# mark1222/arena

Hardware: AMD Instinct MI355X
Metric: mnist_mlp_train_throughput (higher is better)
Workload: dtype fp32; 1 GPU; model=mnist_mlp_784-500-10 (relu, dropout 0.9, adam 1e-3), global_batch=100, parallelism=dp1, impl=fused, exec=hipgraph[full,1 steps/graph]; timed: 2479/2479 graph-replayed, 0 eager, launch=single

## Files before the change

csrc/ops/mlp_kernels.hip:

```cpp
#include "common.h"
#include "adam.h"

#include <algorithm>
#include <cmath>

using namespace arena;

#ifndef ARENA_EXP
#define ARENA_EXP 0
#endif
#ifdef ARENA_TIMELINE
__device__ long long arena::arena_tl_buf[4 * ARENA_TL_BLOCKS * ARENA_TL_SLOTS];
extern "C" hipError_t arena_timeline_read(long long* host, int clear) {
  const size_t bytes = sizeof(long long) * 4 * ARENA_TL_BLOCKS * ARENA_TL_SLOTS;
  hipError_t e = hipDeviceSynchronize();
  if (e == hipSuccess) e = hipMemcpyFromSymbol(host, HIP_SYMBOL(arena::arena_tl_buf), bytes);
  if (e == hipSuccess && clear) {
    void* p = nullptr;
    e = hipGetSymbolAddress(&p, HIP_SYMBOL(arena::arena_tl_buf));
    if (e == hipSuccess) e = hipMemset(p, 0, bytes);
  }
  return e;
}
#endif
// ... 100 lines not shown
#pragma unroll
  for (int r = 0; r < 4; ++r) red[w][4 * g + r][c] = acc[r];
  __syncthreads();
  for (int t = threadIdx.x; t < 256; t += WAVES * 64) {
    const int rr = t >> 4, cc = t & 15;
    const int gm = m0 + rr, gn = n0 + cc;
    if (gm < M && gn < N) {
      float v = 0.f;
#pragma unroll
      for (int ww = 0; ww < WAVES; ++ww) v += red[ww][rr][cc];
      v += bv;
      if (act == 1) v = fmaxf(v, 0.f);
      if (keep_thr != 0xFFFFFFFFu) {
        const uint32_t h = hash4(seed, step, (uint32_t)gm, (uint32_t)gn);
        v = (h < keep_thr) ? v * inv_keep : 0.f;
      }
      Y[(long long)gm * N + gn] = v;
    }
  }
}

constexpr int kHeadMaxT = 16;
constexpr int kHeadMaxC = 16;
constexpr int kHeadStage = 16;

template <int LT, int STAGE, int CB, int TB>
__global__ __launch_bounds__(256) __attribute__((amdgpu_waves_per_eu(1, 4))) void xent_head_kernel(
    const float* __restrict__ H, int M, int D, const float* __restrict__ W2,
    const float* __restrict__ b2, int C, ArenaRowSource lab, float* __restrict__ dlogits,
    float* __restrict__ dZ, float inv_keep, int relu_mask, float loss_scale,
    float* __restrict__ loss_acc, int* __restrict__ correct_acc, int hist_len,
    const long long* hist_step, ArenaCounterOp ctr) {
  extern __shared__ __attribute__((aligned(16))) float ws[];
  const int lane = lane_id();
  const int r = blockIdx.x * 4 + wave_id();
  const int rc = min(r, M - 1);
  const long long pr = gather_row(make_gather(lab), rc);
  int y;
  if constexpr (LT == 1) y = (int)static_cast<const uint8_t*>(lab.ptr)[pr];
  else if constexpr (LT == 2) y = static_cast<const int*>(lab.ptr)[pr];
  else y = (int)static_cast<const long long*>(lab.ptr)[pr];
  float h[TB];
#pragma unroll
  for (int t = 0; t < TB; ++t) h[t] = H[(long long)rc * D + min(lane + 64 * t, D - 1)];
  const int n4 = (D * C) >> 2;
  float4 st[STAGE];
#pragma unroll
  for (int i = 0; i < STAGE; ++i)
    st[i] = reinterpret_cast<const float4*>(W2)[min((int)threadIdx.x + 256 * i, n4 - 1)];
  const float bl = b2 ? b2[min(lane, C - 1)] : 0.f;
  const long long hs = hist_step ? *hist_step : 0;
#pragma unroll
  for (int i = 0; i < STAGE; ++i) {
    const int q = threadIdx.x + 256 * i;
    reinterpret_cast<float4*>(ws)[q < n4 ? q : n4] = st[i];
  }
  counter_op(ctr);
  const int hmask = hist_len - 1;
  const int slot = (int)hs & hmask;
  if (hist_len > 1 && blockIdx.x == 0 && threadIdx.x == 0) {
    const int nxt = (int)(hs + 1) & hmask;
    loss_acc[nxt] = 0.f;
    correct_acc[nxt] = 0;
  }
  __syncthreads();
  if (r >= M) return;
  int jo[TB];
#pragma unroll
  for (int t = 0; t < TB; ++t) {
    const int j = lane + 64 * t;
    jo[t] = min(j, D - 1);
    h[t] = (j < D) ? h[t] : 0.f;
  }

  float lg[CB];
#pragma unroll
  for (int cc = 0; cc < CB; ++cc) {
    const float* wr = ws + min(cc, C - 1) * D;
    float s = 0.f;
#pragma unroll
    for (int t = 0; t < TB; ++t) s += h[t] * wr[jo[t]];
    lg[cc] = s;
  }
#pragma unroll
  for (int cc = 0; cc < CB; ++cc) {
    const float tot = wave_sum_fast(lg[cc]) +
                      __int_as_float(__builtin_amdgcn_readlane(__float_as_int(bl), cc));
    lg[cc] = (cc < C) ? tot : -INFINITY;
  }
  float mx = lg[0];
  int arg = 0;
#pragma unroll
  for (int cc = 1; cc < CB; ++cc) {
    const bool gt = lg[cc] > mx;
    mx = gt ? lg[cc] : mx;
    arg = gt ? cc : arg;
  }
  float se = 0.f;
#pragma unroll
  for (int cc = 0; cc < CB; ++cc) se += (cc < C) ? hw_exp2((lg[cc] - mx) * kLog2e) : 0.f;
  const float lse = mx + hw_log2(se) * kLn2;
  float ly = 0.f;
#pragma unroll
  for (int cc = 0; cc < CB; ++cc) ly = (cc == y) ? lg[cc] : ly;
  if (lane == 0) {
    atomicAdd(&loss_acc[slot], (lse - ly) * loss_scale);
    atomicAdd(&correct_acc[slot], arg == y ? 1 : 0);
  }
  if (dlogits == nullptr) return;

  float gcl[CB];
#pragma unroll
  for (int cc = 0; cc < CB; ++cc)
    gcl[cc] = (cc < C) ? (hw_exp2((lg[cc] - lse) * kLog2e) - (cc == y ? 1.f : 0.f)) * loss_scale
                       : 0.f;
  if (lane < C) {
    float v = 0.f;
#pragma unroll
    for (int cc = 0; cc < CB; ++cc) v = (cc == lane) ? gcl[cc] : v;
    dlogits[(long long)r * C + lane] = v;
  }
  if (dZ == nullptr) return;
  float o[TB];
#pragma unroll
  for (int t = 0; t < TB; ++t) {
    float s = 0.f;
#pragma unroll
    for (int cc = 0; cc < CB; ++cc) s += gcl[cc] * ws[min(cc, C - 1) * D + jo[t]];
    o[t] = relu_mask ? ((h[t] > 0.f) ? s * inv_keep : 0.f) : s;
  }
#pragma unroll
  for (int t = 0; t < TB; ++t) {
    const int j = lane + 64 * t;
    if (j < D) dZ[(long long)r * D + j] = o[t];
  }
}

constexpr int kMaxProblems = 2;
struct WGradArgs {
  ArenaWGradProblem p[kMaxProblems];
  int nprob;
  ArenaAdam adam;
  float grad_scale;
  ArenaCounterOp ctr;
  ArenaHead head;
  int head_block;
};

constexpr int kMC = 128;
constexpr int kXsStride = 80;
constexpr int kXItems = (kMC * 16) / 256;
constexpr int kZItems = (kMC * 4) / 256;
constexpr int kDItems = (kMC * 16) / 256;

__device__ __forceinline__ void lds_barrier() {
  asm volatile("s_waitcnt lgkmcnt(0)" ::: "memory");
  __builtin_amdgcn_s_barrier();
  asm volatile("" ::: "memory");
}

template <int XT>
__device__ __forceinline__ void load_x_items(const ArenaWGradProblem& P, const Gather& gt, int mc0,
                                             int mcn, int k0, float4 (&v)[kXItems]) {
  int prow[kXItems];
#pragma unroll
  for (int i = 0; i < kXItems; ++i) {
    const int t = threadIdx.x + 256 * i;
    prow[i] = gather_row(gt, mc0 + min(t >> 4, mcn - 1));
  }
#pragma unroll
  for (int i = 0; i < kXItems; ++i) {
    const int q = (threadIdx.x + 256 * i) & 15;
    float f[4];
    load4<XT>(P.x, prow[i], min(k0 + 4 * q, P.K - 4), f);
    v[i] = make_float4(f[0], f[1], f[2], f[3]);
  }
}

__device__ __forceinline__ int load_label(const ArenaRowSource& lab, long long pr) {
  if (lab.dtype == 1) return (int)static_cast<const uint8_t*>(lab.ptr)[pr];
  if (lab.dtype == 2) return static_cast<const int*>(lab.ptr)[pr];
  return (int)static_cast<const long long*>(lab.ptr)[pr];
}

template <int SPEC>
struct WSpec {
  static constexpr bool known = SPEC != 0;
  static constexpr int s = SPEC - 1;
  static constexpr int xt = s & 1, hm = (s >> 1) & 3, gather = (s >> 3) & 1, mode = (s >> 4) & 1;
  static constexpr bool sp = known && ((s >> 5) & 1);
};


constexpr int wgrad_spec(int xt, int hm, int gather, int mode, int sp = 0) {
  return 1 + xt + 2 * hm + 8 * gather + 16 * mode + 32 * sp;
}

template <int CB, int SPEC, int LG, int LDT>
__device__ __forceinline__ void wgrad_body(const WGradArgs& args, int pi, float* Xs, float* Zs,
                                           float* Ds, float* W2s, int* Ys, float* B2s) {
  using WS = WSpec<SPEC>;
  const ArenaWGradProblem& P = args.p[pi];
  const ArenaHead& HD = args.head;
  const int local = blockIdx.x - P.block_begin;
  int tn, tk;
  if ((P.tiles_n & 7) == 0 && (P.block_begin & 7) == 0) {
    const int xcd = local & 7, slot = local >> 3;
    tn = xcd + 8 * (slot / P.tiles_k);
    tk = slot % P.tiles_k;
  } else {
    tn = local / P.tiles_k;
    tk = local % P.tiles_k;
  }
  const int n0 = tn * 16, k0 = tk * 64;
  const int lane = lane_id(), w = wave_id();
  const int g = lane >> 4, c = lane & 15;
  const int kk = k0 + 16 * w + c;
  const int kkc = min(kk, P.K - 1);
  const bool bias_wave = (tk == 0) && (w == 0);
  const int mode = WS::known ? WS::mode : P.mode;
  const int xt = WS::known ? WS::xt : P.xt;
  const int hmode = WS::known ? WS::hm : P.hd_mode;
  const bool has_bias = mode == 1 ? P.pB != nullptr : P.gB != nullptr;
  const Gather gt = (WS::known && !WS::gather) ? Gather{nullptr, 0, P.M} : make_gather(P.x);
  const bool zvec = (P.N & 3) == 0;
  ARENA_TL(1, 0);
  int lz;
  asm volatile("v_mov_b32 %0, 0" : "=v"(lz));
  long long hstep_raw = 0, adam_t = 1;
  float adam_lr = args.adam.lr;
  if constexpr (WS::known) {
    if (WS::hm) hstep_raw = *reinterpret_cast<const int*>(HD.step) + lz;
    if (WS::mode == 1) {
      adam_t = *reinterpret_cast<const int*>(args.adam.t_ptr) + lz;
      adam_lr = *args.adam.lr_ptr + __int_as_float(lz);
    }
  } else {
    if (hmode) hstep_raw = *HD.step;
    if (mode == 1) {
      adam_t = args.adam.t_ptr ? *args.adam.t_ptr : 1;
      adam_lr = args.adam.lr_ptr ? *args.adam.lr_ptr : args.adam.lr;
    }
  }
  const float* logits = nullptr;
  long long hstep = 0;

  f32x4 acc = {0.f, 0.f, 0.f, 0.f};
  f32x4 accb = {0.f, 0.f, 0.f, 0.f};
  float pw[4], mw[4], vw[4], pb[4], mb[4], vb[4];
  const int nchunks = WS::known ? 1 : (P.M + kMC - 1) / kMC;
  for (int ci = 0; ci < nchunks; ++ci) {
    const int mc0 = ci * kMC;
    const int mcn = min(kMC, P.M - mc0);
    float4 xv[kXItems];
    if (ARENA_EXP & 2) {
#pragma unroll
      for (int i = 0; i < kXItems; ++i) xv[i] = make_float4(0.5f, 0.25f, 0.f, 1.f);
    } else if (xt == 1) {
      load_x_items<1>(P, gt, mc0, mcn, k0, xv);
    } else {
      load_x_items<0>(P, gt, mc0, mcn, k0, xv);
    }
    ARENA_TL(1, 8);
    float4 zv[kZItems];
    float dv[kDItems];
    float wv = 0.f, bv = 0.f;
    int yv = 0;
    if (hmode == 0) {
#pragma unroll
      for (int i = 0; i < kZItems; ++i) {
        const int t = threadIdx.x + 256 * i;
        const int rr = min(t >> 2, mcn - 1), q = t & 3;
        const int n = n0 + 4 * q;
        const float* srcp = P.dz + (long long)(mc0 + rr) * P.N;
        if (zvec) {
          zv[i] = *reinterpret_cast<const float4*>(srcp + min(n, P.N - 4));
        } else {
          zv[i] = make_float4(srcp[min(n, P.N - 1)], srcp[min(n + 1, P.N - 1)],
                              srcp[min(n + 2, P.N - 1)], srcp[min(n + 3, P.N - 1)]);
        }
      }
    } else {
      const int C = HD.C;
      if ((int)threadIdx.x < kMC) {
        const Gather lg = (LG == 0) ? Gather{nullptr, 0, P.M} : make_gather(HD.lab);
        const long long pr = gather_row(lg, mc0 + min((int)threadIdx.x, mcn - 1));
        if constexpr (LDT == 1) yv = static_cast<const uint8_t*>(HD.lab.ptr)[pr];
        else if constexpr (LDT == 2) yv = static_cast<const int*>(HD.lab.ptr)[pr];
        else yv = load_label(HD.lab, pr);
      }
      {
        const float* b2p = HD.b2 ? HD.b2 : P.hd_w2 ? P.hd_w2 : HD.logits2;
        const float b2v = b2p[min((int)threadIdx.x & 15, C - 1)];
        bv = HD.b2 ? b2v : 0.f;
      }
      if (hmode == 2) {
#pragma unroll
        for (int i = 0; i < kZItems; ++i) {
          const int t = threadIdx.x + 256 * i;
          const int rr = min(t >> 2, mcn - 1), q = t & 3;
          if (ARENA_EXP & 4) zv[i] = make_float4(1.f, 0.f, 1.f, 1.f);
          else zv[i] = *reinterpret_cast<const float4*>(P.hd_h + (long long)(mc0 + rr) * P.N +
                                                        min(n0 + 4 * q, P.N - 4));
        }
        wv = P.hd_w2[(long long)min((int)threadIdx.x >> 4, C - 1) * P.N +
                     min(n0 + ((int)threadIdx.x & 15), P.N - 1)];
      }
      ARENA_TL(1, 9);
      if (mc0 == 0) {
        if constexpr (WS::sp) {
          logits = HD.logits2 + (long long)HD.parity * P.M * HD.C;
          ARENA_TL(1, 1);
        } else {
          if (ARENA_EXP & 16) hstep_raw = 7;
          hstep = hstep_raw + HD.step_off;
          logits = HD.logits2 + (long long)(hstep & 1) * P.M * HD.C;
          ARENA_TL_DEP((int)hstep);
          ARENA_TL(1, 1);
        }
      }
#pragma unroll
      for (int i = 0; i < kDItems; ++i) {
        const int t = threadIdx.x + 256 * i;
        if (ARENA_EXP & 1) dv[i] = 0.01f * (float)(t & 15);
        else dv[i] = logits[(long long)(mc0 + min(t >> 4, mcn - 1)) * C + min(t & 15, C - 1)];
      }
      ARENA_TL(1, 10);
      if (mc0 == 0 && (int)blockIdx.x == args.head_block) {
        if constexpr (WS::sp) hstep = hstep_raw + HD.step_off;
        float* nxt = HD.logits2 + (long long)((hstep + 1) & 1) * P.M * HD.C;
        for (int i = threadIdx.x; i < P.M * HD.C; i += 256) nxt[i] = 0.f;
        if (HD.nr_out != nullptr && (int)threadIdx.x < HD.nr_batch) {
          long long q = mod_fp64((double)(hstep + 1) * (double)HD.nr_batch, HD.nr_len) +
                        (long long)threadIdx.x;
          q = (q >= HD.nr_len) ? q - HD.nr_len : q;
          HD.nr_out[threadIdx.x] = HD.nr_perm[q];
        }
        if (threadIdx.x == 0 && HD.hist_len > 1) {
          const int ns = (int)(hstep + 1) & (HD.hist_len - 1);
          HD.loss_acc[ns] = 0.f;
          HD.correct_acc[ns] = 0;
        }
      }
    }
    if (mc0 == 0 && mode == 1 && (ARENA_EXP & 32)) {
#pragma unroll
      for (int r = 0; r < 4; ++r) { pw[r] = 0.1f; mw[r] = 0.01f; vw[r] = 0.001f; }
#pragma unroll
      for (int r = 0; r < 4; ++r) { pb[r] = 0.1f; mb[r] = 0.01f; vb[r] = 0.001f; }
    } else if (mc0 == 0 && mode == 1) {
#pragma unroll
      for (int r = 0; r < 4; ++r) {
        const long long off = (long long)min(n0 + 4 * g + r, P.N - 1) * P.K + kkc;
        pw[r] = P.pW[off]; mw[r] = P.mW[off]; vw[r] = P.vW[off];
      }
      {
        const float* pbp = has_bias ? P.pB : P.pW;
        const float* mbp = has_bias ? P.mB : P.mW;
        const float* vbp = has_bias ? P.vB : P.vW;
#pragma unroll
        for (int r = 0; r < 4; ++r) {
          const int n = min(n0 + 4 * g + r, P.N - 1);
          pb[r] = pbp[n]; mb[r] = mbp[n]; vb[r] = vbp[n];
        }
      }
    }
#pragma unroll
    for (int i = 0; i < kXItems; ++i) {
      const int t = threadIdx.x + 256 * i;
      const int rr = t >> 4, q = t & 15;
      const float4 o = (k0 + 4 * q < P.K) ? xv[i] : make_float4(0.f, 0.f, 0.f, 0.f);
      *reinterpret_cast<float4*>(&Xs[rr * kXsStride + 4 * q]) = o;
    }
    if (hmode == 0) {
#pragma unroll
      for (int i = 0; i < kZItems; ++i) {
        const int t = threadIdx.x + 256 * i;
        const int rr = t >> 2, q = t & 3;
        const int n = n0 + 4 * q;
        float4 o = zv[i];
        o.x = (n + 0 < P.N) ? o.x : 0.f;
        o.y = (n + 1 < P.N) ? o.y : 0.f;
        o.z = (n + 2 < P.N) ? o.z : 0.f;
        o.w = (n + 3 < P.N) ? o.w : 0.f;
        if (rr >= mcn) o = make_float4(0.f, 0.f, 0.f, 0.f);
        *reinterpret_cast<float4*>(&Zs[rr * 16 + 4 * q]) = o;
      }
    } else {
      const int C = HD.C;
#pragma unroll
      for (int i = 0; i < kDItems; ++i) Ds[threadIdx.x + 256 * i] = dv[i];
      if ((int)threadIdx.x < kMC) Ys[threadIdx.x] = yv;
      if (threadIdx.x < 16) B2s[threadIdx.x] = bv;
      W2s[threadIdx.x] = (((int)threadIdx.x >> 4) < C) ? wv : 0.f;
      lds_barrier();
      ARENA_TL(1, 2);
      float loss = 0.f, corr = 0.f;
      if ((int)threadIdx.x < mcn) {
        float* row = &Ds[threadIdx.x * 16];
        const int y = Ys[threadIdx.x];
        float lgv[CB];
        float mx = -INFINITY;
        int arg = 0;
#pragma unroll
        for (int cc = 0; cc < CB; ++cc) {
          lgv[cc] = row[cc] + B2s[cc];
          const bool better = cc < C && lgv[cc] > mx;
          mx = better ? lgv[cc] : mx;
          arg = better ? cc : arg;
        }
        float pe[CB];
        float se = 0.f;
#pragma unroll
        for (int cc = 0; cc < CB; ++cc) {
          pe[cc] = (cc < C) ? hw_exp2((lgv[cc] - mx) * kLog2e) : 0.f;
          se += pe[cc];
        }
        const float inv = hw_rcp(se);
        const float lse = mx + hw_log2(se) * kLn2;
        float ly = 0.f;
#pragma unroll
        for (int cc = 0; cc < CB; ++cc) {
          ly = (cc == y) ? lgv[cc] : ly;
          row[cc] = (pe[cc] * inv - (cc == y ? 1.f : 0.f)) * HD.loss_scale;
        }
        loss = (lse - ly) * HD.loss_scale;
        corr = (arg == y) ? 1.f : 0.f;
      }
      if ((int)blockIdx.x == args.head_block) {
        const float ls = wave_sum_fast(loss), cs = wave_sum_fast(corr);
        if (lane == 0 && w * 64 < mcn) {
          const int slot = (int)hstep & (HD.hist_len - 1);
          atomicAdd(&HD.loss_acc[slot], ls);
          atomicAdd(&HD.correct_acc[slot], (int)(cs + 0.5f));
        }
      }
      lds_barrier();
      ARENA_TL(1, 3);
#pragma unroll
      for (int i = 0; i < kZItems; ++i) {
        const int t = threadIdx.x + 256 * i;
        const int rr = t >> 2, q = t & 3;
        const int n = n0 + 4 * q;
        float z[4];
        if (hmode == 1) {
          const float4 d4 = *reinterpret_cast<const float4*>(&Ds[rr * 16 + 4 * q]);
          z[0] = d4.x; z[1] = d4.y; z[2] = d4.z; z[3] = d4.w;
        } else {
          z[0] = z[1] = z[2] = z[3] = 0.f;
#pragma unroll
          for (int cc = 0; cc < CB; ++cc) {
            const float d = Ds[rr * 16 + cc];
            const float4 w4 = *reinterpret_cast<const float4*>(&W2s[cc * 16 + 4 * q]);
            z[0] += d * w4.x; z[1] += d * w4.y; z[2] += d * w4.z; z[3] += d * w4.w;
          }
          const float4 hm = zv[i];
          const float ik = P.hd_inv_keep;
          z[0] = hm.x > 0.f ? z[0] * ik : 0.f;
          z[1] = hm.y > 0.f ? z[1] * ik : 0.f;
          z[2] = hm.z > 0.f ? z[2] * ik : 0.f;
          z[3] = hm.w > 0.f ? z[3] * ik : 0.f;
        }
        float4 o = make_float4((n + 0 < P.N) ? z[0] : 0.f, (n + 1 < P.N) ? z[1] : 0.f,
                               (n + 2 < P.N) ? z[2] : 0.f, (n + 3 < P.N) ? z[3] : 0.f);
        if (rr >= mcn) o = make_float4(0.f, 0.f, 0.f, 0.f);
        *reinterpret_cast<float4*>(&Zs[rr * 16 + 4 * q]) = o;
      }
    }
    lds_barrier();
    ARENA_TL(1, 4);
    if (mcn > kMC / 2) {
      f32x4 ch[4] = {acc, {0.f, 0.f, 0.f, 0.f}, {0.f, 0.f, 0.f, 0.f}, {0.f, 0.f, 0.f, 0.f}};
      if (tk == 0) {
        f32x4 chb[4] = {accb, {0.f, 0.f, 0.f, 0.f}, {0.f, 0.f, 0.f, 0.f}, {0.f, 0.f, 0.f, 0.f}};
#pragma unroll
        for (int s = 0; s < kMC / 4; s += 4) {
#pragma unroll
          for (int j = 0; j < 4; ++j) {
            const int m = 4 * (s + j) + g;
            const float a = Zs[m * 16 + c];
            const float b = Xs[m * kXsStride + 16 * w + c];
            ch[j] = mfma_16x16x4(a, b, ch[j]);
            chb[j] = mfma_16x16x4(a, 1.f, chb[j]);
          }
        }
        accb = (chb[0] + chb[1]) + (chb[2] + chb[3]);
      } else {
#pragma unroll
        for (int s = 0; s < kMC / 4; s += 4) {
#pragma unroll
          for (int j = 0; j < 4; ++j) {
            const int m = 4 * (s + j) + g;
            const float a = Zs[m * 16 + c];
            const float b = Xs[m * kXsStride + 16 * w + c];
            ch[j] = mfma_16x16x4(a, b, ch[j]);
          }
        }
      }
      acc = (ch[0] + ch[1]) + (ch[2] + ch[3]);
    } else {
      const int nst = (mcn + 3) >> 2;
      for (int s = 0; s < nst; ++s) {
        const int m = 4 * s + g;
        const float a = Zs[m * 16 + c];
        const float b = Xs[m * kXsStride + 16 * w + c];
        acc = mfma_16x16x4(a, b, acc);
        if (bias_wave) accb = mfma_16x16x4(a, 1.f, accb);
      }
    }
    if (ci + 1 < nchunks) lds_barrier();
  }
  ARENA_TL_DEP(acc[0]);
  ARENA_TL(1, 5);
  AdamCoef co{};
  if (mode == 1) co = adam_coef_tl(args.adam, (float)adam_t, adam_lr);

  if (mode == 0) {
#pragma unroll
    for (int r = 0; r < 4; ++r) {
      const int n = n0 + 4 * g + r;
      if (kk < P.K && n < P.N) P.gW[(long long)n * P.K + kk] = acc[r] * args.grad_scale;
    }
    if (bias_wave && has_bias && c == 0) {
#pragma unroll
      for (int r = 0; r < 4; ++r) {
        const int n = n0 + 4 * g + r;
        if (n < P.N) P.gB[n] = accb[r] * args.grad_scale;
      }
    }
  } else {
#pragma unroll
    for (int r = 0; r < 4; ++r) {
      const int n = n0 + 4 * g + r;
      if (kk < P.K && n < P.N) {
        const long long off = (long long)n * P.K + kk;
        adam_apply(co, acc[r], pw[r], mw[r], vw[r]);
        P.pW[off] = pw[r]; P.mW[off] = mw[r]; P.vW[off] = vw[r];
      }
    }
    if (bias_wave && has_bias && c == 0) {
#pragma unroll
      for (int r = 0; r < 4; ++r) {
        const int n = n0 + 4 * g + r;
        if (n < P.N) {
          adam_apply(co, accb[r], pb[r], mb[r], vb[r]);
          P.pB[n] = pb[r]; P.mB[n] = mb[r]; P.vB[n] = vb[r];
        }
      }
    }
  }
  ARENA_TL(1, 6);
  ARENA_TL_DRAIN();
  ARENA_TL(1, 7);
}

template <int CB, int S0, int S1>
__global__ __launch_bounds__(256) __attribute__((amdgpu_waves_per_eu(2, 4))) void wgrad_grouped_kernel(
    WGradArgs args) {
  __shared__ __attribute__((aligned(16))) float Xs[kMC * kXsStride];
  __shared__ __attribute__((aligned(16))) float Zs[kMC * 16];
  __shared__ __attribute__((aligned(16))) float Ds[kMC * 16];
  __shared__ __attribute__((aligned(16))) float W2s[16 * 16];
  __shared__ int Ys[kMC];
  __shared__ float B2s[16];
  int pi = 0;
#pragma unroll
  for (int i = 1; i < kMaxProblems; ++i)
    if (i < args.nprob && (int)blockIdx.x >= args.p[i].block_begin) pi = i;
  if constexpr (S0 != 0 && S1 != 0) {
    constexpr int LG = WSpec<S0>::gather;
    constexpr int LDT = LG ? 1 : 2;
    if (pi == 0) wgrad_body<CB, S0, LG, LDT>(args, 0, Xs, Zs, Ds, W2s, Ys, B2s);
    else wgrad_body<CB, S1, LG, LDT>(args, 1, Xs, Zs, Ds, W2s, Ys, B2s);
  } else {
    wgrad_body<CB, 0, -1, -1>(args, pi, Xs, Zs, Ds, W2s, Ys, B2s);
  }
  counter_op(args.ctr);
}


template <int XT, int WAVES, int FM>
__global__ __launch_bounds__(WAVES * 64) void mlp_fwd_logits_kernel(
    ArenaRowSource src, const float* __restrict__ W, const float* __restrict__ bias,
    float* __restrict__ Y, int M, int N, int K, uint32_t keep_thr, float inv_keep, uint32_t seed,
    const long long* step_src, const float* __restrict__ W2, float* __restrict__ W2_copy, int C,
    float* __restrict__ logits2, uint8_t* __restrict__ xb, const void* __restrict__ lab_ptr,
    int lab_dtype, int* __restrict__ yb, ArenaCounterOp ctr, const int* __restrict__ rows) {
  constexpr int CH = 8;
  const int lane = lane_id(), w = wave_id();
  const int g = lane >> 4, c = lane & 15;
  const int n0 = blockIdx.x * 16, m0 = blockIdx.y * 16;
  ARENA_TL(0, 0);
  const int rowc = min(m0 + c, M - 1), colc = min(n0 + c, N - 1);
  const float* wrow = W + (long long)colc * K;
  const int nsteps = (K + 15) >> 4;
  const int s0 = (nsteps * w) / WAVES, s1 = (nsteps * (w + 1)) / WAVES;
  const bool publish = (xb != nullptr) && blockIdx.x == 0;
  __shared__ float w2s[16][17];
  __shared__ float hs[16][17];
  __shared__ float red[WAVES][16][17];
  f32x4 acc = {0.f, 0.f, 0.f, 0.f};
  long long stepv;
  long long prow;
  float w2v, bv;
  constexpr bool FAST = FM != 0;
  if constexpr (FAST) {
    int lz;
    asm volatile("v_mov_b32 %0, 0" : "=v"(lz));
    int prow2 = 0;
    if constexpr (FM == 2) prow2 = rows[rowc] + lz;
    const int A = *reinterpret_cast<const int*>(step_src) + lz;
    __builtin_amdgcn_sched_barrier(0);
    float b[CH][4];
#pragma unroll
    for (int i = 0; i < CH; ++i) {
      const int kc = min((s0 + i) * 16 + 4 * g, K - 4);
      const float4 wv = *reinterpret_cast<const float4*>(wrow + kc);
      b[i][0] = wv.x; b[i][1] = wv.y; b[i][2] = wv.z; b[i][3] = wv.w;
    }
    w2v = W2[(long long)min((int)(threadIdx.x >> 4) & 15, C - 1) * N +
             min(n0 + ((int)threadIdx.x & 15), N - 1)];
    bv = bias[min(n0 + ((int)threadIdx.x & 15), N - 1)];
    __builtin_amdgcn_sched_barrier(0);
    if constexpr (FM == 2) {
      prow = prow2;
    } else {
      long long p = mod_fp64((double)A * (double)src.batch, src.idx_len) + rowc;
      p = (p >= src.idx_len) ? p - src.idx_len : p;
      prow = src.idx[p];
    }
    stepv = A;
    ARENA_TL_DEP((int)prow);
    ARENA_TL(0, 1);
    float a[CH][4];
    uint32_t raw[CH];
#pragma unroll
    for (int i = 0; i < CH; ++i) {
      const int kc = min((s0 + i) * 16 + 4 * g, K - 4);
      if constexpr (XT == 1) {
        raw[i] = *reinterpret_cast<const uint32_t*>(static_cast<const uint8_t*>(src.ptr) +
                                                    prow * (long long)src.ld + kc);
#pragma unroll
        for (int j = 0; j < 4; ++j) a[i][j] = (float)((raw[i] >> (8 * j)) & 0xffu) * src.scale;
      } else {
        load4<XT>(src, prow, kc, a[i]);
        raw[i] = 0;
      }
    }
    if constexpr (XT == 1) {
      if (publish && m0 + c < M) {
#pragma unroll
        for (int i = 0; i < CH; ++i) {
          const int k = (s0 + i) * 16 + 4 * g;
          if (s0 + i < s1 && k < K)
            *reinterpret_cast<uint32_t*>(xb + (long long)(m0 + c) * K + k) = raw[i];
        }
      }
    }
#pragma unroll
    for (int i = 0; i < CH; ++i) {
      const bool kv = ((s0 + i) * 16 + 4 * g) < K && (s0 + i) < s1;
#pragma unroll
      for (int j = 0; j < 4; ++j) a[i][j] = kv ? a[i][j] : 0.f;
    }
    f32x4 ch[4] = {acc, {0.f, 0.f, 0.f, 0.f}, {0.f, 0.f, 0.f, 0.f}, {0.f, 0.f, 0.f, 0.f}};
#pragma unroll
    for (int i = 0; i < CH; ++i) {
#pragma unroll
      for (int j = 0; j < 4; ++j) ch[j] = mfma_16x16x4(a[i][j], b[i][j], ch[j]);
    }
    acc = (ch[0] + ch[1]) + (ch[2] + ch[3]);
  } else {
  const Gather gt = make_gather(src);
  stepv = step_src ? *step_src : 0;
  prow = gather_row(gt, rowc);
  ARENA_TL_DEP((int)prow);
  ARENA_TL(0, 1);
  if (publish && w == 0 && g == 0 && m0 + c < M) {
    const int y = (lab_dtype == 1) ? (int)static_cast<const uint8_t*>(lab_ptr)[prow]
                : (lab_dtype == 2) ? static_cast<const int*>(lab_ptr)[prow]
                                   : (int)static_cast<const long long*>(lab_ptr)[prow];
    yb[m0 + c] = y;
  }
  w2v = 0.f;
  bv = 0.f;
  if (threadIdx.x < 256) {
    w2v = W2[(long long)min((int)threadIdx.x >> 4, C - 1) * N + min(n0 + ((int)threadIdx.x & 15), N - 1)];
    bv = bias[min(n0 + ((int)threadIdx.x & 15), N - 1)];
  }
  counter_op(ctr);
// ... 296 lines not shown
    *reinterpret_cast<float4*>(w) = w4;
    *reinterpret_cast<float4*>(m) = m4;
  } else {
    for (int k = 0; k < 4 && j + k < n; ++k) {
      float wk = w[k], mk = m[k];
      sgd32_1(g[k], wk, mk, lr, mu, wd, scale);
      w[k] = wk;
      m[k] = mk;
    }
  }
}

__global__ void lr_schedule_kernel(const long long* __restrict__ seg, int n_seg,
                                   long long* __restrict__ step, float* __restrict__ lr) {
  if (blockIdx.x != 0 || threadIdx.x != 0) return;
  const long long t = *step;
  int k = 0;
  for (int i = 1; i < n_seg; ++i)
    if (t >= seg[4 * i]) k = i;
  const long long b = seg[4 * k], e = seg[4 * k + 1];
  const double lr0 = __longlong_as_double(seg[4 * k + 2]);
  const double lr1 = __longlong_as_double(seg[4 * k + 3]);
  double v = lr1;
  if (k < n_seg - 1) {
    v = lr0;
    if (lr1 != lr0) {
      const double frac = (double)(t - b) / (double)(e - b);
      double rise = (lr1 - lr0) * frac;
      asm volatile("" : "+v"(rise));
      v = lr0 + rise;
    }
  }
  *lr = (float)v;
  *step = t + 1;
}

}

extern "C" {

hipError_t arena_linear_fwd(ArenaRowSource src, const float* W, const float* bias, float* Y, int M,
                            int N, int K, int act, float keep_prob, uint32_t seed,
                            const long long* step_src, hipStream_t stream) {
  uint32_t thr = 0xFFFFFFFFu;
  float inv_keep = 1.f;
  if (keep_prob < 1.f) {
    thr = (uint32_t)((double)keep_prob * 4294967296.0);
    inv_keep = 1.f / keep_prob;
  }
  dim3 grid((N + 15) / 16, (M + 15) / 16);
  if (src.dtype == 1)
    hipLaunchKernelGGL((linear_fwd_kernel<1, 8>), grid, dim3(512), 0, stream, src, W, bias, Y, M,
                       N, K, act, thr, inv_keep, seed, step_src);
  else
    hipLaunchKernelGGL((linear_fwd_kernel<0, 8>), grid, dim3(512), 0, stream, src, W, bias, Y, M,
                       N, K, act, thr, inv_keep, seed, step_src);
  return hipGetLastError();
}

hipError_t arena_mlp_fwd_logits(ArenaRowSource src, const float* W, const float* bias, float* Y,
                                int M, int N, int K, float keep_prob, uint32_t seed,
                                const long long* step_src, const float* W2, float* W2_copy, int C,
                                float* logits2, uint8_t* xb, const void* lab_ptr, int lab_dtype,
                                int* yb, ArenaCounterOp ctr, const int* rows, hipStream_t stream) {
  if (C < 1 || C > 16 || K % 4) return hipErrorInvalidValue;
  uint32_t thr = 0xFFFFFFFFu;
  float inv_keep = 1.f;
  if (keep_prob < 1.f) {
    thr = (uint32_t)((double)keep_prob * 4294967296.0);
    inv_keep = 1.f / keep_prob;
  }
  dim3 grid((N + 15) / 16, (M + 15) / 16);
  const int nsteps = (K + 15) / 16;
  const bool fast = src.dtype == 1 && src.idx != nullptr && src.cursor != nullptr &&
                    src.cursor == step_src && src.cursor_off == 0 && ctr.dst != nullptr &&
                    ctr.src == step_src && xb != nullptr && lab_ptr != nullptr &&
                    (nsteps + 7) / 8 <= 8 && src.idx_len < (1LL << 31);
  if (fast && rows != nullptr)
    hipLaunchKernelGGL((mlp_fwd_logits_kernel<1, 8, 2>), grid, dim3(512), 0, stream, src, W,
                       bias, Y, M, N, K, thr, inv_keep, seed, step_src, W2, W2_copy, C, logits2,
                       xb, lab_ptr, lab_dtype, yb, ctr, rows);
  else if (fast)
    hipLaunchKernelGGL((mlp_fwd_logits_kernel<1, 8, 1>), grid, dim3(512), 0, stream, src, W,
                       bias, Y, M, N, K, thr, inv_keep, seed, step_src, W2, W2_copy, C, logits2,
                       xb, lab_ptr, lab_dtype, yb, ctr, rows);
  else if (src.dtype == 1)
    hipLaunchKernelGGL((mlp_fwd_logits_kernel<1, 8, 0>), grid, dim3(512), 0, stream, src, W,
                       bias, Y, M, N, K, thr, inv_keep, seed, step_src, W2, W2_copy, C, logits2,
                       xb, lab_ptr, lab_dtype, yb, ctr, nullptr);
  else
    hipLaunchKernelGGL((mlp_fwd_logits_kernel<0, 8, 0>), grid, dim3(512), 0, stream, src, W,
                       bias, Y, M, N, K, thr, inv_keep, seed, step_src, W2, W2_copy, C, logits2,
                       nullptr, lab_ptr, lab_dtype, yb, ctr, nullptr);
  return hipGetLastError();
}

hipError_t arena_xent_head(const float* H, int M, int D, const float* W2, const float* b2, int C,
                           ArenaRowSource lab, float* dlogits, float* dZ, float keep_prob,
                           int relu_mask, float loss_scale, float* loss_acc, int* correct_acc,
                           int hist_len, const long long* hist_step, ArenaCounterOp ctr,
                           hipStream_t stream) {
  if (D > 64 * kHeadMaxT || C > kHeadMaxC || D * C > 1024 * kHeadStage || (D * C) % 4)
    return hipErrorInvalidValue;
  const float inv_keep = keep_prob < 1.f ? 1.f / keep_prob : 1.f;
  dim3 grid((M + 3) / 4);
  const size_t smem = sizeof(float) * ((size_t)D * C + 4);
  const bool big = D * C > 1024 * 8;
  const bool small = C <= 10 && D <= 512 && !big;
#define ARENA_HEAD(LT, ST, CB, TB)                                                               \
  hipLaunchKernelGGL((xent_head_kernel<LT, ST, CB, TB>), grid, dim3(256), smem, stream, H, M, D, \
                     W2, b2, C, lab, dlogits, dZ, inv_keep, relu_mask, loss_scale, loss_acc,     \
                     correct_acc, hist_len, hist_step, ctr)
#define ARENA_HEAD_LT(LT)                \
  if (small) ARENA_HEAD(LT, 8, 10, 8);   \
  else if (big) ARENA_HEAD(LT, 16, 16, 16); \
  else ARENA_HEAD(LT, 8, 16, 16);
  switch (lab.dtype) {
    case 1: ARENA_HEAD_LT(1) break;
    case 2: ARENA_HEAD_LT(2) break;
    default: ARENA_HEAD_LT(3)
  }
#undef ARENA_HEAD_LT
#undef ARENA_HEAD
  return hipGetLastError();
}

hipError_t arena_wgrad_grouped(ArenaWGradProblem* probs, int nprob, ArenaAdam adam,
                               float grad_scale, ArenaCounterOp ctr, ArenaHead head,
                               hipStream_t stream) {
  if (nprob < 1 || nprob > kMaxProblems) return hipErrorInvalidValue;
  WGradArgs a;
  int blocks = 0;
  for (int i = 0; i < nprob; ++i) {
    probs[i].tiles_k = (probs[i].K + 63) / 64;
    probs[i].tiles_n = (probs[i].N + 15) / 16;
    probs[i].block_begin = blocks;
    blocks += probs[i].tiles_k * probs[i].tiles_n;
    a.p[i] = probs[i];
  }
  a.nprob = nprob;
  a.head_block = -1;
  for (int i = 0; i < nprob; ++i)
    if (probs[i].hd_mode != 0) { a.head_block = probs[i].block_begin; break; }
  a.adam = adam;
  a.grad_scale = grad_scale;
  a.ctr = ctr;
  a.head = head;
  const bool g0 = probs[0].x.idx != nullptr;
  const bool sp = head.parity == 0 || head.parity == 1;
  const bool mlp_pair = nprob == 2 && head.C <= 10 && probs[0].xt == 1 && probs[0].hd_mode == 2 &&
                        probs[1].xt == 0 && probs[1].hd_mode == 1 && probs[1].x.idx == nullptr &&
                        probs[0].mode == probs[1].mode && probs[0].M <= kMC &&
                        (probs[0].mode == 0 || (adam.t_ptr && adam.lr_ptr)) && head.step &&
                        probs[1].M <= kMC && head.lab.dtype == (g0 ? 1 : 2);
  const dim3 grid(blocks), block(256);
  if (mlp_pair) {
    const int m = probs[0].mode & 1;
#define ARENA_WG_PAIR(G, M, SP)                                                                \
  hipLaunchKernelGGL((wgrad_grouped_kernel<10, wgrad_spec(1, 2, G, M, SP),                     \
                                           wgrad_spec(0, 1, 0, M, SP)>), grid, block, 0, stream, a)
    if (sp) {
      if (g0 == 0 && m == 0) ARENA_WG_PAIR(0, 0, 1);
      else if (g0 == 0 && m == 1) ARENA_WG_PAIR(0, 1, 1);
      else if (g0 == 1 && m == 0) ARENA_WG_PAIR(1, 0, 1);
      else ARENA_WG_PAIR(1, 1, 1);
    } else {
      if (g0 == 0 && m == 0) ARENA_WG_PAIR(0, 0, 0);
      else if (g0 == 0 && m == 1) ARENA_WG_PAIR(0, 1, 0);
      else if (g0 == 1 && m == 0) ARENA_WG_PAIR(1, 0, 0);
      else ARENA_WG_PAIR(1, 1, 0);
    }
#undef ARENA_WG_PAIR
  } else if (head.C <= 10) {
    hipLaunchKernelGGL((wgrad_grouped_kernel<10, 0, 0>), grid, block, 0, stream, a);
  } else {
    hipLaunchKernelGGL((wgrad_grouped_kernel<16, 0, 0>), grid, block, 0, stream, a);
  }
  return hipGetLastError();
}

hipError_t arena_adam_flat(float* P, float* M, float* V, const float* G, long long n,
                           ArenaAdam adam, ArenaCounterOp ctr, hipStream_t stream) {
  if (n % 4) return hipErrorInvalidValue;
  const long long n4 = n / 4;
  const int blocks = (int)std::min<long long>((n4 + 255) / 256, 2048);
  hipLaunchKernelGGL(adam_flat_kernel, dim3(blocks > 0 ? blocks : 1), dim3(256), 0, stream, P, M, V,
                     G, n4, adam, ctr);
  return hipGetLastError();
}

hipError_t arena_sgd_flat(float* P, const float* G, long long n, float lr, const float* lr_ptr,
                          float gscale, hipStream_t stream) {
  if (n % 4) return hipErrorInvalidValue;
  const long long n4 = n / 4;
  const int blocks = (int)std::min<long long>((n4 + 255) / 256, 2048);
  hipLaunchKernelGGL(sgd_flat_kernel, dim3(blocks > 0 ? blocks : 1), dim3(256), 0, stream, P, G, n4,
                     lr, lr_ptr, gscale);
  return hipGetLastError();
}

hipError_t arena_softmax_xent(const float* logits, const long long* labels, int M, int C,
                              float* loss, float* dlogits, float grad_scale, hipStream_t stream) {
  hipLaunchKernelGGL(softmax_xent_kernel, dim3((M + 3) / 4), dim3(256), 0, stream, logits, labels,
                     M, C, loss, dlogits, grad_scale);
  return hipGetLastError();
}

hipError_t arena_mt_copy_scale(float* const* ptrs, const long long* offs, const long long* ns,
                               int count, float* flat, float scale, int dir, hipStream_t stream) {
  for (int base = 0; base < count; base += kMtMax) {
    MtArgs a;
    const int cnt = std::min(kMtMax, count - base);
    int blocks = 0;
    for (int i = 0; i < cnt; ++i) {
      a.ptr[i] = ptrs[base + i];
      a.off[i] = offs[base + i];
      a.n[i] = ns[base + i];
      a.blk_begin[i] = blocks;
      blocks += (int)((ns[base + i] + 1023) / 1024);
    }
    a.blk_begin[cnt] = blocks;
    a.count = cnt;
    if (blocks == 0) continue;
    hipLaunchKernelGGL(mt_copy_scale_kernel, dim3(blocks), dim3(256), 0, stream, a, flat, scale,
                       dir);
    hipError_t e = hipGetLastError();
    if (e != hipSuccess) return e;
  }
  return hipSuccess;
}

hipError_t arena_mt_sgd_master(const void* const* grads, const long long* offs, const long long* ns,
                               int count, float* master, float* mom, void* wbf, float lr,
                               const float* lr_ptr, float mu, float wd, hipStream_t stream) {
  for (int base = 0; base < count; base += kMtMax) {
    MtArgs a;
    const int cnt = std::min(kMtMax, count - base);
    int blocks = 0;
    for (int i = 0; i < cnt; ++i) {
      if (ns[base + i] % 4 || offs[base + i] % 4) return hipErrorInvalidValue;
      a.ptr[i] = const_cast<float*>(reinterpret_cast<const float*>(grads[base + i]));
      a.off[i] = offs[base + i];
      a.n[i] = ns[base + i];
      a.blk_begin[i] = blocks;
      blocks += (int)((ns[base + i] + 1023) / 1024);
    }
    a.blk_begin[cnt] = blocks;
    a.count = cnt;
    if (blocks == 0) continue;
    hipLaunchKernelGGL(mt_sgd_master_kernel, dim3(blocks), dim3(256), 0, stream, a, master, mom,
                       reinterpret_cast<uint16_t*>(wbf), lr, lr_ptr, mu, wd);
    hipError_t e = hipGetLastError();
    if (e != hipSuccess) return e;
  }
  return hipSuccess;
}

hipError_t arena_shard_sgd(const void* grad, int grad_bf16, float* w32, float* mom, void* wbf,
                           long long n, float lr, const float* lr_ptr, float mu, float wd,
                           float scale, hipStream_t stream) {
  if (n % 4 || (grad_bf16 && !wbf)) return hipErrorInvalidValue;
  if (n == 0) return hipSuccess;
  const long long blocks = std::min<long long>((n + 1023) / 1024, 4096);
  if (grad_bf16)
    hipLaunchKernelGGL(shard_sgd_kernel<true>, dim3((unsigned)blocks), dim3(256), 0, stream, grad,
                       w32, mom, reinterpret_cast<uint16_t*>(wbf), n, lr, lr_ptr, mu, wd, scale);
  else
    hipLaunchKernelGGL(shard_sgd_kernel<false>, dim3((unsigned)blocks), dim3(256), 0, stream, grad,
                       w32, mom, nullptr, n, lr, lr_ptr, mu, wd, scale);
  return hipGetLastError();
}

hipError_t arena_mt_sgd_f32(const float* const* grads, const long long* offs, const long long* ns,
                            int count, float* w, float* mom, float lr, const float* lr_ptr,
                            float mu, float wd, float scale, hipStream_t stream) {
  for (int base = 0; base < count; base += kMtMax) {
    MtArgs a;
    const int cnt = std::min(kMtMax, count - base);
    int blocks = 0;
    for (int i = 0; i < cnt; ++i) {
      if (ns[base + i] < 0 || offs[base + i] < 0) return hipErrorInvalidValue;
      a.ptr[i] = const_cast<float*>(grads[base + i]);
      a.off[i] = offs[base + i];
      a.n[i] = ns[base + i];
      a.blk_begin[i] = blocks;
      blocks += (int)((ns[base + i] + 1023) / 1024);
    }
    a.blk_begin[cnt] = blocks;
    a.count = cnt;
    if (blocks == 0) continue;
    hipLaunchKernelGGL(mt_sgd_f32_kernel, dim3(blocks), dim3(256), 0, stream, a, w, mom, lr, lr_ptr,
                       mu, wd, scale);
    hipError_t e = hipGetLastError();
    if (e != hipSuccess) return e;
  }
  return hipSuccess;
}

hipError_t arena_lr_schedule(const long long* seg, int n_seg, long long* step, float* lr,
                             hipStream_t stream) {
  if (n_seg < 1 || n_seg > 64) return hipErrorInvalidValue;
  hipLaunchKernelGGL(lr_schedule_kernel, dim3(1), dim3(1), 0, stream, seg, n_seg, step, lr);
  return hipGetLastError();
}

}
```

Measured before the change: 5.034 million samples/s.

## Transpose wgrad accumulators through LDS for vectorized float4 Adam loads and stores

The weight-gradient epilogue now writes the MFMA accumulator fragments to shared memory and reads them back transposed, so each thread owns four contiguous K elements. The Adam parameter, m and v loads and stores (and the plain gradient store) become 16-byte float4 accesses, and stores use an inline-asm global_store_dwordx4 with the sc1 cache hint. This replaces the earlier strided scalar accesses and is meant to cut memory transactions in the optimizer update. The cost is an extra LDS round trip and a barrier. The fast specialized path now also requires K divisible by 4 and 16-byte-aligned pointers.

After: 5.177 million samples/s (median of 6 runs). +2.8%, better.

```diff
diff --git a/csrc/ops/mlp_kernels.hip b/csrc/ops/mlp_kernels.hip
--- a/csrc/ops/mlp_kernels.hip
+++ b/csrc/ops/mlp_kernels.hip
@@ -276,6 +276,7 @@
 constexpr int kXItems = (kMC * 16) / 256;
 constexpr int kZItems = (kMC * 4) / 256;
 constexpr int kDItems = (kMC * 16) / 256;
+constexpr int kTsStride = 68;
 
 __device__ __forceinline__ void lds_barrier() {
   asm volatile("s_waitcnt lgkmcnt(0)" ::: "memory");
@@ -299,6 +300,17 @@
     load4<XT>(P.x, prow[i], min(k0 + 4 * q, P.K - 4), f);
     v[i] = make_float4(f[0], f[1], f[2], f[3]);
   }
+}
+
+__host__ __device__ inline bool wgrad_vec_ok(const ArenaWGradProblem& P) {
+  const uintptr_t a = P.mode == 1 ? ((uintptr_t)P.pW | (uintptr_t)P.mW | (uintptr_t)P.vW)
+                                  : (uintptr_t)P.gW;
+  return (P.K & 3) == 0 && (a & 15) == 0;
+}
+
+__device__ __forceinline__ void store_f4_wt(float* p, const float4& v) {
+  const f32x4 x = {v.x, v.y, v.z, v.w};
+  asm volatile("global_store_dwordx4 %0, %1, off sc1\n\ts_nop 1" ::"v"(p), "v"(x) : "memory");
 }
 
 __device__ __forceinline__ int load_label(const ArenaRowSource& lab, long long pr) {
@@ -372,6 +384,9 @@
   f32x4 acc = {0.f, 0.f, 0.f, 0.f};
   f32x4 accb = {0.f, 0.f, 0.f, 0.f};
   float pw[4], mw[4], vw[4], pb[4], mb[4], vb[4];
+  float4 pw4 = make_float4(0.f, 0.f, 0.f, 0.f), mw4 = pw4, vw4 = pw4;
+  const int vn = n0 + ((int)threadIdx.x >> 4), vk = k0 + 4 * ((int)threadIdx.x & 15);
+  const bool vec = WS::known || wgrad_vec_ok(P);
   const int nchunks = WS::known ? 1 : (P.M + kMC - 1) / kMC;
   for (int ci = 0; ci < nchunks; ++ci) {
     const int mc0 = ci * kMC;
@@ -473,10 +488,19 @@
 #pragma unroll
       for (int r = 0; r < 4; ++r) { pb[r] = 0.1f; mb[r] = 0.01f; vb[r] = 0.001f; }
     } else if (mc0 == 0 && mode == 1) {
-#pragma unroll
-      for (int r = 0; r < 4; ++r) {
-        const long long off = (long long)min(n0 + 4 * g + r, P.N - 1) * P.K + kkc;
-        pw[r] = P.pW[off]; mw[r] = P.mW[off]; vw[r] = P.vW[off];
+      if (vec) {
+        if constexpr (WS::known) {
+          const long long off = (long long)min(vn, P.N - 1) * P.K + min(vk, P.K - 4);
+          pw4 = *reinterpret_cast<const float4*>(P.pW + off);
+          mw4 = *reinterpret_cast<const float4*>(P.mW + off);
+          vw4 = *reinterpret_cast<const float4*>(P.vW + off);
+        }
+      } else {
+#pragma unroll
+        for (int r = 0; r < 4; ++r) {
+          const long long off = (long long)min(n0 + 4 * g + r, P.N - 1) * P.K + kkc;
+          pw[r] = P.pW[off]; mw[r] = P.mW[off]; vw[r] = P.vW[off];
+        }
       }
       {
         const float* pbp = has_bias ? P.pB : P.pW;
@@ -639,11 +663,27 @@
   AdamCoef co{};
   if (mode == 1) co = adam_coef_tl(args.adam, (float)adam_t, adam_lr);
 
+  float4 g4 = make_float4(0.f, 0.f, 0.f, 0.f);
+  if (vec) {
+#pragma unroll
+    for (int r = 0; r < 4; ++r) Ds[(4 * g + r) * kTsStride + 16 * w + c] = acc[r];
+    lds_barrier();
+    g4 = *reinterpret_cast<const float4*>(&Ds[((int)threadIdx.x >> 4) * kTsStride +
+                                              4 * ((int)threadIdx.x & 15)]);
+  }
+  const bool vok = vk < P.K && vn < P.N;
   if (mode == 0) {
-#pragma unroll
-    for (int r = 0; r < 4; ++r) {
-      const int n = n0 + 4 * g + r;
-      if (kk < P.K && n < P.N) P.gW[(long long)n * P.K + kk] = acc[r] * args.grad_scale;
+    if (vec) {
+      if (vok)
+        store_f4_wt(P.gW + (long long)vn * P.K + vk,
+                 make_float4(g4.x * args.grad_scale, g4.y * args.grad_scale,
+                             g4.z * args.grad_scale, g4.w * args.grad_scale));
+    } else {
+#pragma unroll
+      for (int r = 0; r < 4; ++r) {
+        const int n = n0 + 4 * g + r;
+        if (kk < P.K && n < P.N) P.gW[(long long)n * P.K + kk] = acc[r] * args.grad_scale;
+      }
     }
     if (bias_wave && has_bias && c == 0) {
 #pragma unroll
@@ -653,13 +693,31 @@
       }
     }
   } else {
-#pragma unroll
-    for (int r = 0; r < 4; ++r) {
-      const int n = n0 + 4 * g + r;
-      if (kk < P.K && n < P.N) {
-        const long long off = (long long)n * P.K + kk;
-        adam_apply(co, acc[r], pw[r], mw[r], vw[r]);
-        P.pW[off] = pw[r]; P.mW[off] = mw[r]; P.vW[off] = vw[r];
+    if (vec) {
+      if (vok) {
+        const long long off = (long long)vn * P.K + vk;
+        if constexpr (!WS::known) {
+          pw4 = *reinterpret_cast<const float4*>(P.pW + off);
+          mw4 = *reinterpret_cast<const float4*>(P.mW + off);
+          vw4 = *reinterpret_cast<const float4*>(P.vW + off);
+        }
+        adam_apply(co, g4.x, pw4.x, mw4.x, vw4.x);
+        adam_apply(co, g4.y, pw4.y, mw4.y, vw4.y);
+        adam_apply(co, g4.z, pw4.z, mw4.z, vw4.z);
+        adam_apply(co, g4.w, pw4.w, mw4.w, vw4.w);
+        store_f4_wt(P.pW + off, pw4);
+        store_f4_wt(P.mW + off, mw4);
+        store_f4_wt(P.vW + off, vw4);
+      }
+    } else {
+#pragma unroll
+      for (int r = 0; r < 4; ++r) {
+        const int n = n0 + 4 * g + r;
+        if (kk < P.K && n < P.N) {
+          const long long off = (long long)n * P.K + kk;
+          adam_apply(co, acc[r], pw[r], mw[r], vw[r]);
+          P.pW[off] = pw[r]; P.mW[off] = mw[r]; P.vW[off] = vw[r];
+        }
       }
     }
     if (bias_wave && has_bias && c == 0) {
@@ -1262,7 +1320,8 @@
                         probs[1].xt == 0 && probs[1].hd_mode == 1 && probs[1].x.idx == nullptr &&
                         probs[0].mode == probs[1].mode && probs[0].M <= kMC &&
                         (probs[0].mode == 0 || (adam.t_ptr && adam.lr_ptr)) && head.step &&
-                        probs[1].M <= kMC && head.lab.dtype == (g0 ? 1 : 2);
+                        probs[1].M <= kMC && head.lab.dtype == (g0 ? 1 : 2) &&
+                        wgrad_vec_ok(probs[0]) && wgrad_vec_ok(probs[1]);
   const dim3 grid(blocks), block(256);
   if (mlp_pair) {
     const int m = probs[0].mode & 1;
```
